# saegsali/visual-odometry-project

Measured on AMD Instinct MI355X. Metric: VO frames/sec at 1376x1241, 2k keypoints; pose err vs reference, higher is better.
Workload: dtype f64

## Files before the change

### include/vo_hip.h

```cpp
#ifndef VO_HIP_H
#define VO_HIP_H

#include <stddef.h>
#include <stdint.h>

#ifdef __cplusplus
extern "C" {
#endif

typedef struct vo_ctx vo_ctx;

typedef enum vo_status {
  VO_OK = 0,
  VO_EINVAL = -1,
  VO_ENOMEM = -2,
  VO_EHIP = -3,
  VO_ECAPACITY = -4,
  VO_ETRACKING = -5
} vo_status;


int vo_create(int device, void* stream, vo_ctx** out);
void vo_destroy(vo_ctx* ctx);
const char* vo_last_error(const vo_ctx* ctx);
// ... 229 lines not shown
int vo_ransac_replay(vo_ransac_state* st, const uint8_t* valid, const int32_t* counts, int B,
                     int N, int64_t* n_done, int32_t* best_count, int32_t* best_idx,
                     int idx_offset, int* consumed, int* finished);

typedef struct vo_pipeline vo_pipeline;
typedef struct vo_pipeline_config {
  int32_t H, W, n_frames;
  int32_t n_keypoints, harris_patch, nms_radius;
  double harris_kappa;
  int32_t klt_win, klt_max_level, klt_max_iter, hyp;
  double klt_eps, klt_min_eig, klt_err_threshold;
  double p3p_thr_sq, ransac_outlier_ratio, ransac_confidence;
  int64_t ransac_max_iterations;
  double K[9];
  double Kinv[9];
  int32_t refine_iters;
  int32_t feature_cap;
  double bearing_threshold;
  double redetect_fraction;
  int32_t debug_fault_every;
  int32_t redetect_start_pose;
  double detect_margin;
  int32_t debug_never_detect;
  double detect_losses;
  int32_t sequences;
  int32_t tracker_mode;
  int32_t sift_cap;
  int32_t track_ids;
  double match_ratio;
  int32_t detector;
  int32_t st_block;
  double st_quality;
  double st_min_distance;
} vo_pipeline_config;
typedef struct vo_step_result {
  double R[9], t[3];
  int32_t n_tracked;
  int32_t n_inliers;
  int32_t best_index;
  int32_t hyp_valid;
  int64_t ransac_iterations;
  int32_t draws_consumed;
  int32_t refine_iterations;
  double R_refined[9], t_refined[3];
  double refine_cost;
  int32_t n_features_in;
// ... 209 lines not shown
```

### visual-odometry-project_amd/csrc/harris.hip

```cpp
#include "vo_internal.h"

#pragma clang fp contract(off)

namespace {

constexpr int NT = 256;
constexpr int RX = 64;
constexpr int RY = 32;

struct resp_geom {
  int pr, GW, GWp, GH, IWp, IH;
};
typedef short pk16 __attribute__((ext_vector_type(2)));
__device__ __forceinline__ pk16 as_pk16(unsigned v) { return __builtin_bit_cast(pk16, v); }
__device__ __forceinline__ unsigned as_u32(pk16 v) { return __builtin_bit_cast(unsigned, v); }
__host__ __device__ inline resp_geom response_geometry(int p) {
  resp_geom g;
  g.pr = p >> 1;
  g.GW = RX + 2 * g.pr;
  g.GWp = (g.GW + 3) & ~3;
  g.GH = RY + 2 * g.pr;
  g.IWp = g.GWp + 4;
  g.IH = g.GH + 2;
  return g;
// ... 1334 lines not shown
      VO_HIP_TRY(ctx, hipFuncSetAttribute(reinterpret_cast<const void*>(&harris_response_kernel<0>),
                                          hipFuncAttributeMaxDynamicSharedMemorySize, (int)response_lds_bytes(31)));
      lds_opt_in = true;
    }
    vo_prof_scope ps(ctx, VO_K_HARRIS_RESPONSE);
    if (patch == 9)
      hipLaunchKernelGGL(harris_response_kernel<9>, grid, dim3(NT), lds, ctx->stream, d_img, H, W, patch, kappa,
                         d_scores, img_stride, d_go);
    else
      hipLaunchKernelGGL(harris_response_kernel<0>, grid, dim3(NT), lds, ctx->stream, d_img, H, W, patch, kappa,
                         d_scores, img_stride, d_go);
  }
  return vo_check_launch(ctx, "harris_response_kernel");
}

extern "C" {

int vo_nms_keypoints_dev(vo_ctx* ctx, const double* d_scores, int H, int W, int N, int r, double* d_kp_xy) {
  return vo_nms_keypoints_batch_dev(ctx, d_scores, 1, H, W, N, r, d_kp_xy, 0);
}

}

int vo_nms_keypoints_batch_dev(vo_ctx* ctx, const double* d_scores, int S, int H, int W, int N, int r, double* d_kp_xy,
                               size_t kp_stride, const int* d_go) {
  if (!ctx) return VO_EINVAL;
  VO_REQUIRE(ctx, S >= 1 && S <= 65535, "nms: bad sequence count");
  VO_REQUIRE(ctx, d_scores && d_kp_xy, "nms: null pointer");
  VO_REQUIRE(ctx, H > 0 && W > 0 && (int64_t)H * W < (1ll << 30), "nms: bad map size %dx%d", W, H);
  VO_REQUIRE(ctx, W < 65536 && H < 65536, "nms: map side must be < 65536");
  VO_REQUIRE(ctx, N >= 1 && N <= MAX_N, "nms: N must be in 1..%d", MAX_N);
  VO_REQUIRE(ctx, r >= 0 && r <= 12, "nms: radius must be in 0..12");
  VO_HIP_TRY(ctx, hipSetDevice(ctx->device));
  const unsigned cap = (unsigned)H * (unsigned)W;
  const unsigned cap_c = next_pow2(2u * cap);
  const dim3 grid(vo_cdiv(W, CX), vo_cdiv(H, CY), S);
  const unsigned nblk = grid.x * grid.y;
  const size_t seg_total = (size_t)nblk * SEG;
  const size_t Sz = (size_t)S;
  VO_TRY(vo_ensure(ctx, ctx->nms_keys_l1, Sz * seg_total * 8));
  VO_TRY(vo_ensure(ctx, ctx->nms_idx_l1, Sz * seg_total * 4));
  VO_TRY(vo_ensure(ctx, ctx->nms_keys_a1, Sz * seg_total * 8));
  VO_TRY(vo_ensure(ctx, ctx->nms_idx_a1, Sz * seg_total * 4));
  VO_TRY(vo_ensure(ctx, ctx->nms_cand, Sz * seg_total * 4));
  VO_TRY(vo_ensure(ctx, ctx->nms_segcnt, Sz * nblk * sizeof(uint4)));
  VO_TRY(vo_ensure(ctx, ctx->nms_keys_c, Sz * cap_c * 8));
  VO_TRY(vo_ensure(ctx, ctx->nms_idx_c, Sz * cap_c * 4));
  VO_TRY(vo_ensure(ctx, ctx->nms_sel, Sz * MAX_N * 4));
  if (ctx->nms_hist.cap < Sz * 2 * HIST_TOTAL * 4 || ctx->nms_S != S) {
    VO_TRY(vo_ensure(ctx, ctx->nms_hist, Sz * 2 * HIST_TOTAL * 4));
    VO_HIP_TRY(ctx, hipMemsetAsync(ctx->nms_hist.p, 0, ctx->nms_hist.cap, ctx->stream));
    ctx->nms_S = S;
  }
  if (ctx->nms_rank.cap < Sz * RANK_MAX * 4) {
    VO_TRY(vo_ensure(ctx, ctx->nms_rank, Sz * RANK_MAX * 4));
    VO_HIP_TRY(ctx, hipMemsetAsync(ctx->nms_rank.p, 0, ctx->nms_rank.cap, ctx->stream));
// ... 13 lines not shown
    B.alive = cap;
    B.hist = HIST_TOTAL;
    B.rank = RANK_MAX;
    B.sel = MAX_N;
    B.kp = kp_stride;
  }
  B.go = d_go;
  nms_ctl* ctl = (nms_ctl*)ctx->nms_ctl.p;

  unsigned long long* keys_l1 = (unsigned long long*)ctx->nms_keys_l1.p;
  unsigned long long* keys_a1 = (unsigned long long*)ctx->nms_keys_a1.p;
  unsigned* idx_l1 = (unsigned*)ctx->nms_idx_l1.p;
  unsigned* idx_a1 = (unsigned*)ctx->nms_idx_a1.p;
  unsigned long long* keys_c = (unsigned long long*)ctx->nms_keys_c.p;
  unsigned* idx_c = (unsigned*)ctx->nms_idx_c.p;
  unsigned* cand = (unsigned*)ctx->nms_cand.p;
  uint4* segcnt = (uint4*)ctx->nms_segcnt.p;
  unsigned* alive = (unsigned*)ctx->nms_alive.p;
  ctx->nms_parity ^= 1;
  unsigned* hist = (unsigned*)ctx->nms_hist.p + (size_t)ctx->nms_parity * Sz * HIST_TOTAL;
  unsigned* hist_other = (unsigned*)ctx->nms_hist.p + (size_t)(1 - ctx->nms_parity) * Sz * HIST_TOTAL;
  unsigned* rank = (unsigned*)ctx->nms_rank.p;
  hipStream_t st = ctx->stream;
  {
    bool& lds_opt_in = ctx->lds_opt_in[1];
    if (!lds_opt_in) {
      const int max_dyn = (int)candidates_lds_bytes(12);
      VO_HIP_TRY(ctx, hipFuncSetAttribute(reinterpret_cast<const void*>(&nms_candidates_kernel<5>),
                                          hipFuncAttributeMaxDynamicSharedMemorySize, max_dyn));
      VO_HIP_TRY(ctx, hipFuncSetAttribute(reinterpret_cast<const void*>(&nms_candidates_kernel<0>),
                                          hipFuncAttributeMaxDynamicSharedMemorySize, max_dyn));
      lds_opt_in = true;
    }
    vo_prof_scope ps(ctx, VO_K_NMS_CANDIDATES);
    const size_t lds = candidates_lds_bytes(r);
    if (r == 5)
      hipLaunchKernelGGL(nms_candidates_kernel<5>, grid, dim3(NT), lds, st, d_scores, H, W, r, keys_l1, idx_l1,
                         keys_a1, idx_a1, segcnt, hist, ctl, B);
    else
      hipLaunchKernelGGL(nms_candidates_kernel<0>, grid, dim3(NT), lds, st, d_scores, H, W, r, keys_l1, idx_l1,
                         keys_a1, idx_a1, segcnt, hist, ctl, B);
  }
  VO_TRY(vo_check_launch(ctx, "nms_candidates_kernel"));
  ctx->nms_alive_dirty = true;
  {
    vo_prof_scope ps(ctx, VO_K_NMS_COMPACT);
    hipLaunchKernelGGL(nms_compact_kernel, dim3(nblk, S), dim3(NT), 0, st, keys_l1, idx_l1, keys_a1, idx_a1, segcnt,
                       cand, keys_c, idx_c, alive, ctl, cap_c, hist, hist_other, N, B);
  }
  VO_TRY(vo_check_launch(ctx, "nms_compact_kernel"));
  const size_t round_lds = (size_t)((CX + 2 * r) | 1) * ((CY + 2 * r) + CY) * 4;
  {
    vo_prof_scope ps(ctx, VO_K_NMS_ROUND);
    const dim3 g(nblk, S), b(RT);
    if (r == 5)
      hipLaunchKernelGGL((nms_round_kernel<5, true>), g, b, round_lds, st, d_scores, alive, segcnt, cand, keys_c,
                         idx_c, ctl, cap_c, H, W, r, (int)grid.x, B);
    else
      hipLaunchKernelGGL((nms_round_kernel<0, true>), g, b, round_lds, st, d_scores, alive, segcnt, cand, keys_c,
                         idx_c, ctl, cap_c, H, W, r, (int)grid.x, B);
  }
  VO_TRY(vo_check_launch(ctx, "nms_round_kernel"));
  {
    vo_prof_scope ps(ctx, VO_K_NMS_RANK);
    hipLaunchKernelGGL(nms_rank_kernel, dim3(RK_BLOCKS, S), dim3(NT), 0, st, keys_c, idx_c, ctl, rank, alive, segcnt,
                       cand, nblk, B);
  }
// ... 146 lines not shown
```

### visual-odometry-project_amd/csrc/pipeline.h

```cpp
#pragma once

#include <linux/futex.h>
#include <sys/prctl.h>
#include <sys/syscall.h>
#include <time.h>
#include <unistd.h>

#include <atomic>
#include <chrono>
#include <cmath>
#include <cstdlib>
#include <string>
#include <mutex>
#include <thread>
#include <vector>

#include "vo_state.h"
#include "state_device.h"

struct vo_pipeline_boot;

struct vo_pipeline {
  vo_ctx* ctx = nullptr;
  vo_ctx* det = nullptr;
  vo_ctx* trk = nullptr;
  hipEvent_t evKlt[2] = {nullptr, nullptr}, evRegroup[2] = {nullptr, nullptr};
  vo_pipeline_config cfg;
  std::vector<vo_cam> cams;
  vo_cam* d_cams = nullptr;
  std::vector<char> idle;
  vo_pcg64 seed_rng;
  int n_levels = 1, cap = 0, words = 0, S = 1;
  size_t px = 0, pyr_bytes = 0;
  uint8_t* d_img = nullptr;
  uint8_t* d_pyr = nullptr;
  double* d_kp = nullptr;
  double* d_scores[2] = {nullptr, nullptr};
  int* d_det_go = nullptr;
  float* d_st_xy = nullptr;
  int32_t* d_st_n = nullptr;
  int32_t* d_det_cnt = nullptr;
  int st_rounds = 0;
  double detect_limit = 0.0;
  double detect_losses = 2.5;
  hipEvent_t evPyr[3] = {nullptr, nullptr, nullptr}, evDet[3] = {nullptr, nullptr, nullptr};
  std::vector<uint8_t*> h_img;
  std::vector<hipEvent_t> evImg;
  hipStream_t up_stream = nullptr;
  std::vector<hipEvent_t> evUp;
  std::vector<char> pinned, plain_used;
  std::vector<int> n_pinned;
  struct lens_t {
    bool on = false, have_raw = false;
    double dist[5] = {0, 0, 0, 0, 0}, K_raw[9] = {0, 0, 0, 0, 0, 0, 0, 0, 0};
  };
  std::vector<lens_t> lens;
  uint8_t* d_raw[2] = {nullptr, nullptr};
  uint8_t* h_bgr = nullptr;
  hipEvent_t evBgr = nullptr;
  int prepared_idx = -1, prepared_slot = -1;
  int slot = 0, det_flip = 0, prev_frame = -1;
  vo_feat F[2];
  void* feat_mem = nullptr;
  int cur = 0;
  vo_seq_ctl* d_ctl = nullptr;
  float *d_next = nullptr, *d_err = nullptr;
  uint8_t* d_status = nullptr;
// ... 144 lines not shown
  }
}

static inline vo_cam make_cam(const double* K, const double* Kinv) {
  vo_cam c;
  memcpy(c.K, K, sizeof(c.K));
  if (Kinv) {
    memcpy(c.Kinv, Kinv, sizeof(c.Kinv));
  } else {
    const double fx = K[0], fy = K[4], cx = K[2], cy = K[5];
    const double ki[9] = {1.0 / fx, 0.0, -cx / fx, 0.0, 1.0 / fy, -cy / fy, 0.0, 0.0, 1.0};
    memcpy(c.Kinv, ki, sizeof(ki));
  }
  return c;
}

#define VO_PIPE_INTERNAL __attribute__((visibility("hidden")))
VO_PIPE_INTERNAL void worker_main(vo_pipeline* p);
VO_PIPE_INTERNAL int worker_idle(vo_pipeline* p);
VO_PIPE_INTERNAL int prime(vo_pipeline* p, bool wait = true, int q0 = 0, int Sn = 0);
VO_PIPE_INTERNAL void vo_pipeline_boot_free(vo_pipeline* p);
VO_PIPE_INTERNAL void vo_structure_loop_free(vo_pipeline* p);
VO_PIPE_INTERNAL int vo_structure_loop_requeue(vo_pipeline* p, int q, long k);
VO_PIPE_INTERNAL int enqueue_detection(vo_pipeline* p, int frame, int s, bool force, char* err_buf = nullptr, int q0 = 0, int Sn = 0);
```

### visual-odometry-project_amd/csrc/pipeline.hip

```cpp
#include "pipeline.h"

#pragma clang fp contract(off)

namespace {

hipError_t mset(hipStream_t st, void* dst, int v, size_t bytes) {
  hipError_t e = hipMemsetAsync(dst, v, bytes, st);
  return e != hipSuccess ? e : hipStreamSynchronize(st);
}

uint32_t next_pow2(uint64_t v) {
  uint32_t r = 1;
  while (r < v) r <<= 1;
  return r;
}

vo_feat carve(char*& q, int cap, int S, bool ids) {
  vo_feat f;
  auto take = [&](size_t bytes) {
    void* r = q;
    q += (bytes * S + 255) & ~size_t(255);
    return r;
  };
  f.kp = (float*)take((size_t)cap * 8);
// ... 170 lines not shown
  }
  const int cap = cfg->feature_cap > 0 ? cfg->feature_cap : 2 * cfg->n_keypoints;
  VO_REQUIRE(ctx, cap >= cfg->n_keypoints && cap <= 32768, "pipeline: feature_cap must be in n_keypoints..32768");
  VO_HIP_TRY(ctx, hipSetDevice(ctx->device));
  vo_pipeline* p = new (std::nothrow) vo_pipeline();
  if (!p) return VO_ENOMEM;
  p->ctx = ctx;
  p->cfg = *cfg;
  p->cap = cap;
  p->words = vo_cdiv(cap, 64);
  p->S = cfg->sequences > 0 ? cfg->sequences : 1;
  p->cfg.sequences = p->S;
  const int S = p->S;
  if (p->cfg.bearing_threshold == 0.0) p->cfg.bearing_threshold = 0.0075;
  if (p->cfg.redetect_fraction == 0.0) p->cfg.redetect_fraction = 0.8;
  if (p->cfg.detect_margin == 0.0) p->cfg.detect_margin = 0.01;
  if (p->cfg.detect_losses <= 0.0) p->cfg.detect_losses = 2.5;
  if (p->cfg.st_block == 0) p->cfg.st_block = 7;
  if (p->cfg.st_quality == 0.0) p->cfg.st_quality = 0.01;
  if (p->cfg.st_min_distance == 0.0) p->cfg.st_min_distance = 8.0;
  p->detect_losses = p->cfg.detect_losses;
  p->detect_limit = p->cfg.detect_margin < 0.0 ? -1.0 : p->cfg.redetect_fraction + p->cfg.detect_margin;
  if (p->cfg.debug_never_detect) p->detect_limit = 0.0;
  {
    bool given = false;
    for (double v : cfg->Kinv) given |= v != 0.0;
    p->cams.assign((size_t)p->S, make_cam(cfg->K, given ? cfg->Kinv : nullptr));
  }
  p->idle.assign((size_t)p->S, 0);
  memset(&p->seed_rng, 0, sizeof(p->seed_rng));
  int rc = VO_OK;
  void* side = getenv("VO_ONE_STREAM") ? (void*)ctx->stream : nullptr;
  {
    const char* sc = getenv("VO_SIDE_CUS");
    p->side_cfg = vo_stream_cfg_parse(sc, getenv("VO_STREAM_PRIORITY"));
    if (!sc && p->S <= 2 && p->detect_limit >= 0.0 && !side && cfg->tracker_mode == 0) {
      hipDeviceProp_t prop;
      if (hipGetDeviceProperties(&prop, ctx->device) == hipSuccess && prop.multiProcessorCount >= 128) {
        p->side_cfg.cu_lo = 32;
        p->side_cfg.cu_hi = prop.multiProcessorCount - 1;
      }
    }
    if (!side && side_pool_evicts()) side_evict_except(ctx->device, p->side_cfg);
    for (vo_ctx** c : {&p->trk, &p->det})
      if ((side ? vo_create_stream(ctx->device, side, p->side_cfg, c) : side_take(ctx->device, p->side_cfg, c)) != VO_OK)
        rc = vo_set_error(ctx, VO_EHIP, "pipeline: cannot create the side streams");
// ... 357 lines not shown
```

### visual-odometry-project_amd/csrc/pipeline_step.hip

```cpp
#include "pipeline.h"

#pragma clang fp contract(off)

namespace {

__global__ __launch_bounds__(64) void detect_decide_kernel(const vo_seq_ctl* __restrict__ ctl, int S, double limit, int n_det,
                                                           int force, int* __restrict__ go, double losses) {
  const int q = blockIdx.x * 64 + threadIdx.x;
  if (q >= S) return;
  if (ctl[q].fault & VO_FAULT_IDLE) {
    go[q] = 0;
    return;
  }
  const int n2 = ctl[q].n2;
  const int lost = max(ctl[q].n_in - (ctl[q].redetected ? (n_det < 0 ? ctl[q].num_features : n_det) : 0) - n2, 0);
  go[q] = (force || limit < 0.0 || (limit > 0.0 && (double)n2 - losses * (double)lost < (double)ctl[q].num_features * limit)) ? 1 : 0;
}

__global__ void ctl_resume_kernel(vo_seq_ctl* __restrict__ ctl) {
  ctl->fault = 0;
  ctl->n_p3p = ctl->n_tri;
}

__global__ __launch_bounds__(256) void sift_kp_f64_kernel(const float* __restrict__ rows, const int* __restrict__ n, int cap,
// ... 45 lines not shown
}

void copy_prof(vo_ctx* q, const vo_ctx* from) {
  q->prof_on = from->prof_on;
  q->prof_kernel = from->prof_kernel;
  q->prof_every = from->prof_every;
}

void sync_prof(vo_pipeline* p) {
  for (vo_ctx* q : {p->det, p->trk}) copy_prof(q, p->ctx);
}

}

static int launch_error(vo_pipeline* p, char* err_buf, int rc, const char* what, const char* detail) {
  if (err_buf) {
    snprintf(err_buf, 256, "%s: %s", what, detail);
    return rc;
  }
  return vo_set_error(p->ctx, rc, "%s: %s", what, detail);
}


int enqueue_detection(vo_pipeline* p, int frame, int s, bool force, char* err_buf, int q0, int Sn) {
  const vo_pipeline_config& c = p->cfg;
  if (Sn <= 0) Sn = p->S - q0;
  p->det_flip ^= 1;
  vo_ctx* det = p->det;
  double* scores = p->d_scores[p->det_flip];
  det->nms_kp_f32 = nullptr;
  int* go = p->d_det_go + (size_t)s * p->S + q0;
  bool wait_ok = hipStreamWaitEvent(det->stream, p->evImg[frame], 0) == hipSuccess;
  if (wait_ok && p->n_pinned[frame] > 0) wait_ok = hipStreamWaitEvent(det->stream, p->evUp[frame], 0) == hipSuccess;
  if (!wait_ok) return launch_error(p, err_buf, VO_EHIP, "detection", "hipStreamWaitEvent failed");
  hipLaunchKernelGGL(detect_decide_kernel, dim3(vo_cdiv(Sn, 64)), dim3(64), 0, det->stream, p->d_ctl + q0, Sn, p->detect_limit,
                     c.detector == 1 ? -1 : c.n_keypoints, force ? 1 : 0, go, p->detect_losses);
  int rc = vo_check_launch(det, "detect_decide_kernel");
  if (c.detector == 1) {
    vo_prof_scope ps(det, VO_K_SHI_TOMASI_CHAIN);
    const int N = c.n_keypoints;
    float* xy = p->d_st_xy + (size_t)q0 * N * 2;
    int32_t *n = p->d_st_n + q0, *over = p->d_st_n + p->S + q0;
    if (rc == VO_OK)
      rc = vo_good_features_batch_gated_dev(det, p->img(q0, frame), p->img_stride(), Sn, c.H, c.W, nullptr, 0, N, c.st_quality,
                                            c.st_min_distance, c.st_block, xy, (size_t)N, n, over, nullptr, p->st_rounds,
                                            VO_GFB_CANDIDATES, go);
    if (rc == VO_OK) {
      hipLaunchKernelGGL(st_close_kernel, dim3(vo_cdiv(N, 256), Sn), dim3(256), 0, det->stream, (const float*)xy, (size_t)N * 2,
                         (const int32_t*)n, (const int32_t*)over, (const int*)go, N, p->kp(q0, s), p->det_stride(),
                         p->d_det_cnt + (size_t)s * p->S + q0);
      rc = vo_check_launch(det, "st_close_kernel");
    }
    if (rc == VO_OK && hipEventRecord(p->evDet[s], det->stream) != hipSuccess) rc = VO_EHIP;
    return rc != VO_OK ? launch_error(p, err_buf, rc, "detection", vo_last_error(det)) : VO_OK;
  }
  if (rc == VO_OK)
    rc = vo_harris_response_batch_dev(det, p->img(q0, frame), p->img_stride(), Sn, c.H, c.W, c.harris_patch, c.harris_kappa,
                                      scores, go);
  if (rc == VO_OK)
    rc = vo_nms_keypoints_batch_dev(det, scores, Sn, c.H, c.W, c.n_keypoints, c.nms_radius, p->kp(q0, s), p->det_stride(),
                                    go);
  if (rc == VO_OK && hipEventRecord(p->evDet[s], det->stream) != hipSuccess) rc = VO_EHIP;
  return rc != VO_OK ? launch_error(p, err_buf, rc, "detection", vo_last_error(det)) : VO_OK;
}

static int enqueue_pyramid(vo_pipeline* p, int frame, int s, int q0 = 0, int Sn = 0) {
  if (s == p->prepared_slot) p->prepared_idx = p->prepared_slot = -1;
  if (p->n_pinned[frame] > 0 && hipStreamWaitEvent(p->trk->stream, p->evUp[frame], 0) != hipSuccess)
    return vo_set_error(p->ctx, VO_EHIP, "pyramid: hipStreamWaitEvent failed");
  const vo_pipeline_config& c = p->cfg;
  if (Sn <= 0) Sn = p->S - q0;
  for (int a = q0; a < q0 + Sn;) {
    if (p->idle[a]) {
      ++a;
      continue;
    }
    int b = a + 1;
    while (b < q0 + Sn && !p->idle[b]) ++b;
    const int rc = vo_pyramid_build_batch_dev(p->trk, p->img(a, frame), p->img_stride(), b - a, c.H, c.W, p->n_levels,
                                              p->pyr(a, s), p->pyr_stride());
    if (rc != VO_OK) return vo_set_error(p->ctx, rc, "pyramid: %s", vo_last_error(p->trk));
    a = b;
  }
  VO_HIP_TRY(p->ctx, hipEventRecord(p->evPyr[s], p->trk->stream));
// ... 100 lines not shown
  }
  return VO_OK;
}

static int enqueue_pose_half(vo_pipeline* p, const vo_pipeline::flight_t& f, int q0, int Sn, unsigned seq);

static int enqueue_chain(vo_pipeline* p, const vo_pipeline::flight_t& f, bool first_half_only, int debug_fault_every,
                         int q0, int Sn, unsigned seq) {
  vo_ctx* ctx = p->ctx;
  const vo_pipeline_config& c = p->cfg;
  const size_t q = (size_t)q0;
  const vo_feat A = vo_feat_seq(p->F[f.fcur], q), B = vo_feat_seq(p->F[1 - f.fcur], q);
  vo_seq_ctl* ctl = p->d_ctl + q0;
  VO_HIP_TRY(ctx, hipStreamWaitEvent(ctx->stream, p->evKlt[f.k & 1], 0));
  vo_append ap;
  ap.det_kp = p->kp(q0, f.a);
  ap.det_stride = p->det_stride();
  ap.n_det = c.n_keypoints;
  ap.frac = c.redetect_fraction;
  ap.pose_mode = c.redetect_start_pose;
  ap.debug_fault_every = debug_fault_every > 0 ? debug_fault_every : 0;
  ap.det_go = p->d_det_go + (size_t)f.a * p->S + q0;
  ap.nf_par = (int)(f.k & 1);
  if (p->d_det_cnt) ap.n_det_dev = p->d_det_cnt + (size_t)f.a * p->S + q0;
  ctx->next_stop = p->evRegroup[f.k & 1];
  VO_TRY(vo_state_regroup_klt(ctx, ctl, A, B, p->d_next + q * p->cap * 2, p->d_status + q * p->cap, p->d_err + q * p->cap,
                              (float)c.klt_err_threshold, ap, p->cap, Sn));
  if (first_half_only) return VO_OK;
  return enqueue_pose_half(p, f, q0, Sn, seq);
}

static int enqueue_pose_half(vo_pipeline* p, const vo_pipeline::flight_t& f, int q0, int Sn, unsigned seq) {
  vo_ctx* ctx = p->ctx;
  const int debug_pose_fault = p->pose_fault_hook && p->cfg.debug_fault_every < 0 ? -p->cfg.debug_fault_every : 0;
  const vo_pipeline_config& c = p->cfg;
  const size_t q = (size_t)q0;
  const vo_feat B = vo_feat_seq(p->F[1 - f.fcur], q);
  vo_seq_ctl* ctl = p->d_ctl + q0;
  vo_hyp_batch hb;
  hb.S = Sn;
  hb.X = (size_t)p->cap * 3;
  hb.x = (size_t)p->cap * 2;
  hb.raws = p->ring_len;
  hb.ctl = sizeof(vo_seq_ctl);
  hb.cam = reinterpret_cast<const double*>(p->d_cams + q);
  hb.cam_stride = sizeof(vo_cam) / sizeof(double);
// ... 106 lines not shown
  (void)hipSetDevice(p->ctx->device);
  unsigned seen = 0;
  long idle = 0;
  double idle_since = 0.0;
  for (;;) {
    if (p->job_posted.load(std::memory_order_acquire) == seen) {
      if (p->quit.load(std::memory_order_acquire)) return;
      if (idle == 0) idle_since = now_s();
      if ((++idle & 63) != 0 || now_s() - idle_since < p->spin_s) {
        __builtin_ia32_pause();
      } else {
        p->worker_asleep.store(1, std::memory_order_seq_cst);
        if (p->job_posted.load(std::memory_order_seq_cst) == seen && !p->quit.load(std::memory_order_seq_cst))
          futex_wait(&p->job_posted, seen);
        p->worker_asleep.store(0, std::memory_order_seq_cst);
        idle = 0;
      }
      continue;
    }
    idle = 0;
    const vo_pipeline::flight_t j = p->jobs[seen & 3];
    const int rc = p->cfg.tracker_mode == 1   ? enqueue_sift(p, j, p->worker_err)
                   : p->cfg.tracker_mode == 2 ? enqueue_harris_front(p, j, p->worker_err)
                                              : enqueue_detection(p, j.next_idx, j.b, false, p->worker_err);
    if (rc != VO_OK) p->worker_rc = rc;
    ++seen;
    p->job_done.store(seen, std::memory_order_release);
  }
}

static int worker_check(vo_pipeline* p) {
  if (p->worker_rc != VO_OK) {
    const int rc = p->worker_rc;
    p->worker_rc = VO_OK;
    return vo_set_error(p->ctx, rc, "%s", p->worker_err);
  }
  return VO_OK;
}

int worker_idle(vo_pipeline* p) {
  if (p->threads_budget < 2) return VO_OK;
  const unsigned posted = p->job_posted.load(std::memory_order_relaxed);
  wait_until(50e-6, [&] { return p->job_done.load(std::memory_order_acquire) == posted; });
  return worker_check(p);
}

int prime(vo_pipeline* p, bool wait, int q0, int Sn) {
// ... 105 lines not shown
      const unsigned my = p->job_posted.load(std::memory_order_relaxed);
      wait_until(50e-6, [&] { return (int)(p->job_done.load(std::memory_order_acquire) - my) >= 0; });
      VO_TRY(worker_check(p));
      sync_prof(p);
      if (detect_early) post_job(p, f);
    } else {
      sync_prof(p);
    }
    double tn = now_s();
    p->dbg_part[0] += tn - tq;
    tq = tn;
    const bool have_pyr = p->prepared_idx == next_idx && p->prepared_slot == f.b;
    p->prepared_idx = p->prepared_slot = -1;
    VO_TRY(enqueue_tracker(p, f, !have_pyr, 0, p->S));
    tn = now_s();
    p->dbg_part[1] += tn - tq;
    tq = tn;
    for (int q = 0; q < p->S; ++q) VO_TRY(ensure_raws(p, q));
    tn = now_s();
    p->dbg_part[2] += tn - tq;
    tq = tn;
    VO_TRY(enqueue_chain(p, f, false, c.debug_fault_every, 0, p->S, f.seq));
    for (int q = 0; q < p->S; ++q) p->slot_seq[(size_t)f.rslot * p->S + q] = f.seq;
    if (p->threads_budget < 2) VO_TRY(enqueue_detection(p, f.next_idx, f.b, false));
    else if (!detect_early) post_job(p, f);
    p->dbg_part[3] += now_s() - tq;
    p->flight[p->n_flight++] = f;
  }
  ++p->steps_submitted;
  p->slot = f.b;
  p->cur = 1 - f.fcur;
  p->prev_frame = next_idx;
  p->dbg_submit += now_s() - t_in;
  ++p->dbg_steps;
  return VO_OK;
}

}

static void record_words(const vo_step_result* rec, unsigned seq, unsigned* head, unsigned* tail) {
  const unsigned* dw = reinterpret_cast<const unsigned*>(rec);
  unsigned x = 0u, y = 0u;
  for (size_t k = 0; k + 2 < sizeof(*rec) / 4; ++k) {
    x ^= dw[k];
    y += vo_state_dev::record_mix(dw[k], (int)k);
  }
  *head = seq ^ x;
// ... 288 lines not shown
```

### visual-odometry-project_amd/csrc/state.hip

```cpp
#include <cmath>

#include "dlt_device.h"
#include "state_device.h"

#pragma clang fp contract(off)

namespace {

constexpr int RG_T = 1024;


using namespace vo_state_dev;

__device__ __forceinline__ unsigned long long block_scan_excl(unsigned long long v, unsigned long long* s_wave,
                                                              unsigned long long* total) {
  const int lane = threadIdx.x & 63, wv = threadIdx.x >> 6, nw = blockDim.x >> 6;
  unsigned long long inc = v;
#pragma unroll
  for (int off = 1; off < 64; off <<= 1) {
    const unsigned long long o = __shfl_up(inc, off);
    if (lane >= off) inc += o;
  }
  if (lane == 63) s_wave[wv] = inc;
  __syncthreads();
// ... 253 lines not shown
    r_e[u] = err[min(j, capm)];
    r_st[u] = A.state[min(j, pitm)];
  }
  const int jo = start + tid, jq = min(jo, pitm), jx = min(jo, capm);
  double o_land[3], o_track[2], o_kp[2], o_pose[12];
  const float o_nx = next_xy[2 * jx];
  const float o_ny = next_xy[2 * jx + 1];
#pragma unroll
  for (int k = 0; k < 3; ++k) o_land[k] = A.land[3 * jq + k];
#pragma unroll
  for (int k = 0; k < 2; ++k) {
    o_track[k] = A.track[2 * jq + k];
    o_kp[k] = A.kp64[2 * jq + k];
  }
#pragma unroll
  for (int k = 0; k < 12; ++k) o_pose[k] = A.pose[(size_t)k * A.pitch + jq];
  int2 o_id = make_int2(0, 0);
  if (IDS) o_id = A.ids[jq];
  auto key_of = [&](int j) -> int {
    const int jc = min(j, n_in - 1), js = min(j, max(n - 1, 0));
    const int s8 = status[jc];
    const float e = err[jc];
    const int st_raw = A.state[js];
    const int keep = (int)(j < n_in) & (int)(s8 != 0) & (int)(e < err_thr);
    const int st = j < n ? st_raw : 0;
    return keep ? (st == 2 ? 0 : (st == 1 ? 1 : 2)) : 3;
  };
  unsigned long long c_all = 0ull, c_before = 0ull;
  int my_key = 3;
  for (int base0 = 0; base0 < n_in; base0 += 256 * RG_U) {
    int keys[RG_U];
#pragma unroll
    for (int u = 0; u < RG_U; ++u) {
      const int j = base0 + u * 256 + tid;
      if (base0 == 0) {
        const int keep = (int)(j < n_in) & (int)(r_s8[u] != 0) & (int)(r_e[u] < err_thr);
        const int st = j < n ? r_st[u] : 0;
        keys[u] = keep ? (st == 2 ? 0 : (st == 1 ? 1 : 2)) : 3;
      } else {
        keys[u] = key_of(j);
      }
    }
#pragma unroll
    for (int u = 0; u < RG_U; ++u) {
      const int base = base0 + u * 256;
      const int key = keys[u];
      if (base == start) my_key = key;
      if (key < 3) {
        const unsigned long long one = 1ull << (21 * key);
        c_all += one;
        if (base < start) c_before += one;
      }
    }
  }
#pragma unroll
  for (int off = 32; off >= 1; off >>= 1) {
    c_all += __shfl_xor(c_all, off);
    c_before += __shfl_xor(c_before, off);
  }
// ... 52 lines not shown
      B.state[dst] = 1;
      B.land[3 * dst] = B.land[3 * dst + 1] = B.land[3 * dst + 2] = dnan();
      B.track[2 * dst] = (double)(float)ap.det_kp[2 * d];
      B.track[2 * dst + 1] = (double)(float)ap.det_kp[2 * d + 1];
#pragma unroll
      for (int k = 0; k < 12; ++k)
        B.pose[(size_t)k * B.pitch + dst] = ap.pose_mode ? ctl->T_wc[k] : ((k == 0 || k == 5 || k == 10) ? 1.0 : 0.0);
    }
  }
  if (blockIdx.x == 0 && tid == 0) {
    ctl->n_in = n_in;
    ctl->redetected = redetect ? 1 : 0;
    ctl->det_ran = ap.det_go ? ap.det_go[blockIdx.y] : 1;
    if (ap.n_det_dev) {
      const int nf_next = redetect ? n_det : nf;
      ctl->nf[ap.nf_par ^ 1] = nf_next;
      ctl->num_features = nf_next;
    }
    if (IDS) {
      ctl->next_id[ap.nf_par ^ 1] = nid + (n_in - n);
      ctl->id_step[ap.nf_par ^ 1] = step_k + 1;
    }
    ctl->n2 = T0 + T1 + T2;
    ctl->n_tri = T0;
    ctl->n_mat = T1;
    ctl->n_new = T2;
    const int few = T0 < 8 ? VO_FAULT_FEW_LANDMARKS : 0;
    ctl->n_p3p = few ? 0 : T0;
    ctl->few = few;
  }
}


__global__ __launch_bounds__(256) void state_candidates_kernel(vo_seq_ctl* __restrict__ ctl, vo_feat B,
                                                               const unsigned long long* __restrict__ best_mask,
                                                               const vo_cam* __restrict__ cams, double bearing_thr, int use_refined,
                                                               int words) {
  if (blockIdx.y != 0) {
    const size_t q = blockIdx.y;
    ctl += q;
    B = vo_feat_seq(B, q);
    best_mask += q * (size_t)words;
  }
  const vo_cam& cam = cams[blockIdx.y];
  if (ctl->fault) return;
  const int tid = threadIdx.x;
// ... 409 lines not shown
```

### visual-odometry-project_amd/csrc/state_device.h

```cpp
#pragma once
#include <cstddef>
#include "vo_state.h"

#pragma clang fp contract(off)

namespace vo_state_dev {

__device__ __forceinline__ double dnan() { return __longlong_as_double(0x7ff8000000000000ll); }

__device__ __forceinline__ void rigid_inverse_3x4(const double* T, double* Ti) {
#pragma unroll
  for (int r = 0; r < 3; ++r) {
#pragma unroll
    for (int c = 0; c < 3; ++c) Ti[4 * r + c] = T[4 * c + r];
    Ti[4 * r + 3] = -(T[r] * T[3] + T[4 + r] * T[7] + T[8 + r] * T[11]);
  }
}

__device__ __forceinline__ void k_times(const double* K, const double* T, double* C) {
#pragma unroll
  for (int r = 0; r < 3; ++r)
#pragma unroll
    for (int c = 0; c < 4; ++c) C[4 * r + c] = K[3 * r] * T[c] + K[3 * r + 1] * T[4 + c] + K[3 * r + 2] * T[8 + c];
}

__host__ __device__ inline long long table_lookup(const double* table, int len, long long max_it, double orat) {
  int lo = 0, hi = len;
  while (lo < hi) {
    const int mid = (lo + hi) >> 1;
    if (table[1 + mid] <= orat) lo = mid + 1;
    else hi = mid;
// ... 331 lines not shown
```

### visual-odometry-project_amd/csrc/vo_internal.h

```cpp
#pragma once
#include <hip/hip_runtime.h>
#include <hip/hip_ext.h>

#include <cstdarg>
#include <cstdint>
#include <cstdio>
#include <cstdlib>
#include <cstring>
#include <vector>

#include "vo_hip.h"

struct vo_buf {
  void* p = nullptr;
  size_t cap = 0;
};

struct vo_prof_slot {
  double total_ms = 0.0;
  int64_t launches = 0;
};

struct vo_prof_pair {
  int k;
// ... 4 lines not shown
  int device = 0;
  hipStream_t stream = nullptr;
  bool own_stream = false;
  char err[512] = {0};
  hipEvent_t next_stop = nullptr;

  bool prof_on = false;
  int prof_kernel = -1;
  int prof_every = 1;
  unsigned prof_seen[VO_K_COUNT] = {0};
  vo_prof_slot prof[VO_K_COUNT];
  std::vector<hipEvent_t> ev_free;
  typedef vo_prof_pair pending_ev;
  std::vector<pending_ev> ev_pending;

  vo_buf img, img2, scores, kp, desc;
  vo_buf nms_keys_l1, nms_idx_l1, nms_keys_a1, nms_idx_a1;
  vo_buf nms_keys_c, nms_idx_c;
  vo_buf nms_hist, nms_ctl, nms_sel, nms_cand, nms_alive, nms_segcnt, nms_rank;
  bool nms_alive_dirty = false;
  int nms_parity = 0;
  int nms_S = 0;
  float* nms_kp_f32 = nullptr;
  vo_buf scratch[16];
  vo_buf match_arrived;
  int match_last_path = -1;
  bool lds_opt_in[2] = {false, false};
  hipStream_t aux_stream = nullptr;
  hipStream_t aux_stream2 = nullptr;
  std::vector<hipEvent_t> aux_events;
  vo_buf sift_arena;
  void* h_pin = nullptr;
  size_t h_pin_cap = 0;
  int64_t bytes_h2d = 0, bytes_d2h = 0;
  vo_buf f8_ctl, f8_raws, f8_F, f8_counts, f8_risky, f8_masks, f8_table, f8_samples;
  std::vector<double> f8_table_host;
  double f8_table_conf = 0.0;
  vo_buf ba_work, ba_match;
};

template <class K, class... A>
inline void vo_launch_stop(vo_ctx* ctx, K kernel, dim3 grid, dim3 block, size_t lds, hipStream_t st, A... args) {
  if (ctx->next_stop) {
    hipExtLaunchKernelGGL(kernel, grid, block, (unsigned)lds, st, nullptr, ctx->next_stop, 0, args...);
    ctx->next_stop = nullptr;
  } else {
// ... 164 lines not shown
  int32_t* best = nullptr;
};
int vo_essential_hypotheses_dev(vo_ctx* ctx, const double* d_x1, const double* d_x2, int N, const double* K1, const double* K2,
                                const int32_t* samples, int Hyp, int error_kind, double threshold, const vo_e5_work& w,
                                int32_t* best_count, int32_t* best_sol, uint8_t* valid);
int vo_essential_ransac_dev(vo_ctx* ctx, const double* d_x1, const double* d_x2, int N, const double* K1, const double* K2,
                            int error_kind, double threshold, double outlier_ratio, double confidence, int64_t max_iterations,
                            vo_pcg64* rng, double* d_E, uint8_t* d_inl, int64_t* iterations, int32_t* best_count);
int vo_triangulate_dlt_ndev(vo_ctx* ctx, const double* d_x1, const double* d_x2, const int32_t* d_n, int n_cap,
                            const double* d_C1, const double* d_C2, double* d_X);
int vo_refine_pose_ndev(vo_ctx* ctx, const double* d_X, const double* d_x, int N, const int32_t* d_n, const double* K,
                        const uint8_t* d_mask8, const uint64_t* d_mask_bits, const double* d_Rt0, int max_iter,
                        double* d_out14, unsigned tag);
struct vo_klt_source {
  const int32_t* n = nullptr;
  const int32_t* num_features = nullptr;
  double frac = 0.0;
  const double* det_kp = nullptr;
  int n_det = 0;
  unsigned long long* ts = nullptr;
  const int* det_go = nullptr;
  const int32_t* n_det_dev = nullptr;
};
struct vo_klt_batch {
  int S = 1;
  size_t pyr = 0;
  size_t xy = 0;
  size_t out = 0;
  size_t ctl = 0;
  size_t det = 0;
};
int vo_klt_track_ndev(vo_ctx* ctx, const uint8_t* d_prev, const uint8_t* d_prev_pyr, const uint8_t* d_next,
                      const uint8_t* d_next_pyr, int H, int W, int n_levels, const float* d_prev_xy, int N,
                      const int32_t* d_n, int win, int max_iter, double eps, double min_eig, float* d_next_xy,
                      uint8_t* d_status, float* d_err, const vo_klt_source* src = nullptr,
                      const vo_klt_batch* batch = nullptr, double fb_max = 0.0, float* d_fb = nullptr);
int vo_pyramid_build_batch_dev(vo_ctx* ctx, const uint8_t* d_img, size_t img_stride, int S, int H, int W, int n_levels,
                               uint8_t* d_pyr, size_t pyr_stride);
int vo_harris_response_batch_dev(vo_ctx* ctx, const uint8_t* d_img, size_t img_stride, int S, int H, int W, int patch,
                                 double kappa, double* d_scores, const int* d_go = nullptr);
int vo_nms_keypoints_batch_dev(vo_ctx* ctx, const double* d_scores, int S, int H, int W, int N, int r, double* d_kp_xy,
                               size_t kp_stride, const int* d_go = nullptr);
```

### visual-odometry-project_amd/csrc/vo_state.h

```cpp
#pragma once
#include "vo_internal.h"

struct vo_feat {
  float* kp;
  double* kp64;
  uint8_t* state;
  uint8_t* cand;
  double* land;
  double* track;
  double* pose;
  int pitch;
  int2* ids = nullptr;
};

__host__ __device__ inline vo_feat vo_feat_seq(vo_feat F, size_t q) {
  const size_t n = q * (size_t)F.pitch;
  F.kp += 2 * n;
  F.kp64 += 2 * n;
  F.state += n;
  F.cand += n;
  F.land += 3 * n;
  F.track += 2 * n;
  F.pose += 12 * n;
  if (F.ids) F.ids += n;
// ... 20 lines not shown
  int32_t n2, n_tri, n_mat, n_new;
  int32_t n_p3p;
  int32_t fault;
  int32_t step;
  int32_t solve_flag;
  int32_t few;
  int32_t cont;
  int64_t n_iterations;
  double outlier_ratio;
  uint64_t raw_pos;
  int64_t n_iterations0;
  double outlier_ratio0;
  int32_t best_idx, best_count, consumed, hyp_valid;
  int64_t n_done;
  int32_t n_cand, n_dropped, n_land, done;
  int32_t n_pend, pad_pend;
  double best_pose[12];
  double refined[16];
  double T_cw[12], T_wc[12], T_cw_prev[12], T_wc_prev[12], T_in_cw[12], T_in_wc[12];
  unsigned long long ts[8];
  int32_t nf[2];
  int32_t next_id[2];
  int32_t id_step[2];
};

struct vo_cam {
  double K[9], Kinv[9];
};

struct vo_append {
  const double* det_kp;
  size_t det_stride;
  int n_det;
  double frac;
  int pose_mode;
  int debug_fault_every;
  const int* det_go;
  const int32_t* n_det_dev = nullptr;
  int nf_par = 0;
};

struct vo_replay_args {
  const uint8_t* valid;
  const int32_t* counts;
  const double *R, *t;
  const unsigned long long* masks;
  int words, hyp;
  const double* table;
  int table_len;
  long long max_it;
  unsigned long long* best_mask;
};

struct vo_pose_job {
  vo_seq_ctl* ctl;
  vo_replay_args rp;
  int do_replay;
  vo_feat B;
  const vo_cam* cam;
  double bearing_thr;
  int max_iter;
  int tail;
// ... 33 lines not shown
```

### visual-odometry-project_amd/vo/_native.py

```python
import ctypes as C
import atexit
import os
import threading
import weakref

import numpy as np

_LIB_PATH = os.path.join(os.path.dirname(os.path.abspath(__file__)), "lib", "libvo_hip.so")

VO_OK, VO_EINVAL, VO_ENOMEM, VO_EHIP, VO_ECAPACITY, VO_ETRACKING = 0, -1, -2, -3, -4, -5
_CODES = {VO_EINVAL: "VO_EINVAL", VO_ENOMEM: "VO_ENOMEM", VO_EHIP: "VO_EHIP", VO_ECAPACITY: "VO_ECAPACITY",
          VO_ETRACKING: "VO_ETRACKING"}

K_HARRIS_RESPONSE, K_NMS_CANDIDATES, K_NMS_THRESHOLD, K_NMS_COMPACT, K_NMS_SELECT = 0, 1, 2, 3, 4
K_PATCH_DESC, K_PYR_DOWN, K_KLT_TRACK, K_DLT, K_P3P_SOLVE, K_P3P_SCORE, K_REPROJ, K_MATCH = 5, 6, 7, 8, 9, 10, 11, 12
K_SHI_TOMASI_CHAIN = 27
K_WINDOW_BA, K_WINDOW_BUILD = 28, 29
K_TWOVIEW_HYP, K_TWOVIEW_SCORE = 30, 31
K_WINDOW_STRUCTURE = 32
K_LOOP_RECORD, K_LOOP_JOIN, K_LOOP_WRITE = 33, 34, 35
K_BRIEF_DESCRIBE, K_HAMMING_KNN2 = 36, 37
K_COUNT = 38


# ... 24 lines not shown
        st["state"]["state"] = (self.state_hi << 64) | self.state_lo
        st["state"]["inc"] = (self.inc_hi << 64) | self.inc_lo
        st["has_uint32"] = int(self.has_uint32)
        st["uinteger"] = int(self.uinteger)
        gen.bit_generator.state = st


class RansacState(C.Structure):
    _fields_ = [("outlier_ratio", C.c_double), ("confidence", C.c_double), ("max_iterations", C.c_int64),
                ("n_iterations", C.c_int64), ("s", C.c_int32), ("adaptive", C.c_int32)]


class PipelineConfig(C.Structure):
    _fields_ = [("H", C.c_int32), ("W", C.c_int32), ("n_frames", C.c_int32),
                ("n_keypoints", C.c_int32), ("harris_patch", C.c_int32), ("nms_radius", C.c_int32),
                ("harris_kappa", C.c_double),
                ("klt_win", C.c_int32), ("klt_max_level", C.c_int32), ("klt_max_iter", C.c_int32), ("hyp", C.c_int32),
                ("klt_eps", C.c_double), ("klt_min_eig", C.c_double), ("klt_err_threshold", C.c_double),
                ("p3p_thr_sq", C.c_double), ("ransac_outlier_ratio", C.c_double), ("ransac_confidence", C.c_double),
                ("ransac_max_iterations", C.c_int64),
                ("K", C.c_double * 9), ("Kinv", C.c_double * 9), ("refine_iters", C.c_int32), ("feature_cap", C.c_int32),
                ("bearing_threshold", C.c_double), ("redetect_fraction", C.c_double),
                ("debug_fault_every", C.c_int32), ("redetect_start_pose", C.c_int32), ("detect_margin", C.c_double),
                ("debug_never_detect", C.c_int32), ("detect_losses", C.c_double), ("sequences", C.c_int32),
                ("tracker_mode", C.c_int32), ("sift_cap", C.c_int32), ("track_ids", C.c_int32),
                ("match_ratio", C.c_double),
                ("detector", C.c_int32), ("st_block", C.c_int32), ("st_quality", C.c_double),
                ("st_min_distance", C.c_double)]


class StepResult(C.Structure):
    _fields_ = [("R", C.c_double * 9), ("t", C.c_double * 3), ("n_tracked", C.c_int32), ("n_inliers", C.c_int32),
                ("best_index", C.c_int32), ("hyp_valid", C.c_int32), ("ransac_iterations", C.c_int64),
                ("draws_consumed", C.c_int32), ("refine_iterations", C.c_int32),
                ("R_refined", C.c_double * 9), ("t_refined", C.c_double * 3), ("refine_cost", C.c_double),
                ("n_features_in", C.c_int32), ("redetected", C.c_int32), ("n_triangulated", C.c_int32),
                ("n_candidates", C.c_int32), ("n_dropped", C.c_int32), ("n_landmarks", C.c_int32),
                ("fault", C.c_int32), ("recovered", C.c_int32), ("detector_ran", C.c_int32), ("reserved", C.c_int32),
                ("raw_pos", C.c_uint64), ("T_wc", C.c_double * 12),
                ("ts", C.c_uint64 * 8), ("seq_head", C.c_uint32), ("seq_tail", C.c_uint32)]

    def pose_world_cam(self):
        return np.vstack([np.array(self.T_wc).reshape(3, 4), [0.0, 0.0, 0.0, 1.0]])

    @property
    def idle(self):
        return self.n_features_in == -1
# ... 1165 lines not shown
```

### visual-odometry-project_amd/vo/_pipeline.py

```python
import ctypes as C

import numpy as np


def _ptr(a):
    return a.ctypes.data_as(C.c_void_p) if a is not None else None


def _c(a, dtype):
    return np.ascontiguousarray(a, dtype=dtype)


def _as_4x4(pose):
    pose = np.asarray(pose, np.float64)
    if pose.shape == (3, 4):
        pose = np.vstack([pose, [0.0, 0.0, 0.0, 1.0]])
    return np.ascontiguousarray(pose)


DETECTORS = {"harris": 0, "shi-tomasi": 1}

TRACK_ROW = np.dtype([("id", "<i4"), ("born", "<i4"), ("x", "<f4"), ("y", "<f4"), ("state", "<i4"), ("candidate", "<i4"),
                      ("X", "<f8"), ("Y", "<f8"), ("Z", "<f8")])
TRACK_HEADER = np.dtype([("n", "<i4"), ("step", "<i4"), ("next_id", "<i4"), ("seq", "<i4")])
# ... 3 lines not shown
    n = step = next_id = seq = 0

    def __array_finalize__(self, obj):
        for k in ("n", "step", "next_id", "seq"):
            setattr(self, k, getattr(obj, k, 0))

    @classmethod
    def from_bytes(cls, raw, cap):
        raw = np.ascontiguousarray(raw, np.uint8)
        head = raw[:16].view(TRACK_HEADER)[0]
        m = max(0, min(int(head["n"]), int(cap)))
        rec = raw[16:16 + 48 * m].view(TRACK_ROW).copy().view(cls)
        rec.n, rec.step, rec.next_id, rec.seq = (int(head[k]) for k in ("n", "step", "next_id", "seq"))
        return rec


class Pipeline:
    def __init__(self, ctx, H, W, n_frames, K, n_keypoints=2000, harris_patch=9, harris_kappa=0.09, nms_radius=5,
                 klt_win=15, klt_max_level=2, klt_max_iter=10, klt_eps=0.03, klt_min_eig=1e-4,
                 klt_err_threshold=100.0, hyp=1000, p3p_threshold=1.0, outlier_ratio=0.9, confidence=0.99,
                 max_iterations=1000, seed=2023, refine_iters=0, feature_cap=0, bearing_threshold=0.0075,
                 redetect_fraction=0.8, debug_fault_every=0, redetect_start_pose="identity", sequences=1,
                 detect_margin=0.01, debug_never_detect=0, detect_losses=2.5, tracker="klt", sift_cap=0, match_ratio=0.0,
                 detector="harris", st_quality=0.0, st_min_distance=0.0, st_block=0, track_ids=False):
        from vo import _native
        self.ctx = ctx
        self.cfg = _native.PipelineConfig()
        c = self.cfg
        c.H, c.W, c.n_frames = H, W, n_frames
        c.n_keypoints, c.harris_patch, c.nms_radius, c.harris_kappa = n_keypoints, harris_patch, nms_radius, harris_kappa
        c.klt_win, c.klt_max_level, c.klt_max_iter, c.hyp = klt_win, klt_max_level, klt_max_iter, hyp
        c.klt_eps, c.klt_min_eig, c.klt_err_threshold = klt_eps, klt_min_eig, klt_err_threshold
        c.p3p_thr_sq = p3p_threshold
        c.ransac_outlier_ratio, c.ransac_confidence = outlier_ratio, confidence
        c.ransac_max_iterations = -1 if max_iterations is None or max_iterations == np.inf else int(max_iterations)
        c.refine_iters = int(refine_iters)
        c.feature_cap = int(feature_cap)
        c.bearing_threshold = float(bearing_threshold)
        c.redetect_fraction = float(redetect_fraction)
        c.debug_fault_every = int(debug_fault_every)
        c.redetect_start_pose = {"identity": 0, "current": 1}[redetect_start_pose]
        c.sequences = int(sequences)
        c.detect_margin = float(detect_margin)
        c.debug_never_detect = int(debug_never_detect)
        c.detect_losses = float(detect_losses)
        c.tracker_mode = {"klt": 0, "sift": 1, "harris": 2}[tracker]
        c.sift_cap = int(sift_cap)
        c.match_ratio = float(match_ratio)
        c.detector = DETECTORS[detector]
        c.st_quality, c.st_min_distance, c.st_block = float(st_quality), float(st_min_distance), int(st_block)
        c.track_ids = 1 if track_ids else 0
        self.track_ids = bool(track_ids)
        self.detector = detector
        self.tracker = tracker
        self.sequences = int(sequences)
        K = np.asarray(K, np.float64).reshape(3, 3)
        self.K = K
        for i, v in enumerate(K.reshape(9)):
            c.K[i] = v
        for i, v in enumerate(np.linalg.inv(K).reshape(9)):
            c.Kinv[i] = v
        h = C.c_void_p()
        ctx._chk(ctx._lib.vo_pipeline_create(ctx._h, C.byref(c), C.byref(h)))
        self._h = h
        self._pinned_src = {}
        ctx._pipelines.add(self)
        self.cap = ctx._lib.vo_pipeline_feature_cap(self._h)
        self.seed(np.random.default_rng(seed))

    def close(self):
        if getattr(self, "_h", None):
            if getattr(self, "_loop", None):
                self._loop.close()
            self.ctx._lib.vo_pipeline_destroy(self._h)
# ... 291 lines not shown
```

Baseline: 10920.

## Cancel speculative keypoint detection on device once tracking count confirms no redetect

Adds a device-side recheck kernel that runs during the NMS stage of speculative detection. It reads a tagged tracked-feature count, written atomically by the regroup kernel, and clears the per-sequence go flag when the tracked count is no longer below the redetect fraction. Downstream NMS compact and round kernels can then skip work for detections that are not needed. The cost is extra tiny kernel launches, a new control field, and cross-stream relaxed atomics whose timing determines whether any skipping happens.

```diff
diff --git a/include/vo_hip.h b/include/vo_hip.h
--- a/include/vo_hip.h
+++ b/include/vo_hip.h
@@ -275,6 +275,7 @@
   int32_t redetect_start_pose;
   double detect_margin;
   int32_t debug_never_detect;
+  int32_t detect_confirm;
   double detect_losses;
   int32_t sequences;
   int32_t tracker_mode;
diff --git a/visual-odometry-project_amd/csrc/harris.hip b/visual-odometry-project_amd/csrc/harris.hip
--- a/visual-odometry-project_amd/csrc/harris.hip
+++ b/visual-odometry-project_amd/csrc/harris.hip
@@ -1380,6 +1380,28 @@
 
 }
 
+namespace {
+
+__global__ __launch_bounds__(64) void det_recheck_kernel(vo_det_recheck rc, int S) {
+  const int q = blockIdx.x * 64 + threadIdx.x;
+  if (q >= S || !rc.go[q]) return;
+  const unsigned long long word = __hip_atomic_load(
+      reinterpret_cast<const unsigned long long*>(reinterpret_cast<const char*>(rc.tag) + (size_t)q * rc.stride), __ATOMIC_RELAXED,
+      __HIP_MEMORY_SCOPE_AGENT);
+  if ((unsigned)(word >> 32) != rc.want) return;
+  const int m = (int)(unsigned)(word & 0xffffffffull);
+  const int nf = *reinterpret_cast<const int32_t*>(reinterpret_cast<const char*>(rc.num_features) + (size_t)q * rc.stride);
+  if (!((double)m < (double)nf * rc.frac)) rc.go[q] = 0;
+}
+
+int launch_recheck(vo_ctx* ctx, const vo_det_recheck* rc, int S) {
+  if (!rc || !rc->go) return VO_OK;
+  hipLaunchKernelGGL(det_recheck_kernel, dim3(vo_cdiv(S, 64)), dim3(64), 0, ctx->stream, *rc, S);
+  return vo_check_launch(ctx, "det_recheck_kernel");
+}
+
+}
+
 int vo_nms_keypoints_batch_dev(vo_ctx* ctx, const double* d_scores, int S, int H, int W, int N, int r, double* d_kp_xy,
                                size_t kp_stride, const int* d_go) {
   if (!ctx) return VO_EINVAL;
@@ -1390,6 +1412,8 @@
   VO_REQUIRE(ctx, N >= 1 && N <= MAX_N, "nms: N must be in 1..%d", MAX_N);
   VO_REQUIRE(ctx, r >= 0 && r <= 12, "nms: radius must be in 0..12");
   VO_HIP_TRY(ctx, hipSetDevice(ctx->device));
+  const vo_det_recheck* recheck = ctx->nms_recheck;
+  ctx->nms_recheck = nullptr;
   const unsigned cap = (unsigned)H * (unsigned)W;
   const unsigned cap_c = next_pow2(2u * cap);
   const dim3 grid(vo_cdiv(W, CX), vo_cdiv(H, CY), S);
@@ -1449,6 +1473,7 @@
   unsigned* hist_other = (unsigned*)ctx->nms_hist.p + (size_t)(1 - ctx->nms_parity) * Sz * HIST_TOTAL;
   unsigned* rank = (unsigned*)ctx->nms_rank.p;
   hipStream_t st = ctx->stream;
+  VO_TRY(launch_recheck(ctx, recheck, S));
   {
     bool& lds_opt_in = ctx->lds_opt_in[1];
     if (!lds_opt_in) {
@@ -1470,6 +1495,7 @@
   }
   VO_TRY(vo_check_launch(ctx, "nms_candidates_kernel"));
   ctx->nms_alive_dirty = true;
+  VO_TRY(launch_recheck(ctx, recheck, S));
   {
     vo_prof_scope ps(ctx, VO_K_NMS_COMPACT);
     hipLaunchKernelGGL(nms_compact_kernel, dim3(nblk, S), dim3(NT), 0, st, keys_l1, idx_l1, keys_a1, idx_a1, segcnt,
diff --git a/visual-odometry-project_amd/csrc/pipeline.h b/visual-odometry-project_amd/csrc/pipeline.h
--- a/visual-odometry-project_amd/csrc/pipeline.h
+++ b/visual-odometry-project_amd/csrc/pipeline.h
@@ -43,6 +43,7 @@
   int st_rounds = 0;
   double detect_limit = 0.0;
   double detect_losses = 2.5;
+  bool confirm_on = false;
   hipEvent_t evPyr[3] = {nullptr, nullptr, nullptr}, evDet[3] = {nullptr, nullptr, nullptr};
   std::vector<uint8_t*> h_img;
   std::vector<hipEvent_t> evImg;
@@ -233,4 +234,5 @@
 VO_PIPE_INTERNAL void vo_pipeline_boot_free(vo_pipeline* p);
 VO_PIPE_INTERNAL void vo_structure_loop_free(vo_pipeline* p);
 VO_PIPE_INTERNAL int vo_structure_loop_requeue(vo_pipeline* p, int q, long k);
-VO_PIPE_INTERNAL int enqueue_detection(vo_pipeline* p, int frame, int s, bool force, char* err_buf = nullptr, int q0 = 0, int Sn = 0);
+VO_PIPE_INTERNAL int enqueue_detection(vo_pipeline* p, int frame, int s, bool force, char* err_buf = nullptr, int q0 = 0, int Sn = 0,
+                                       unsigned recheck = 0u);
diff --git a/visual-odometry-project_amd/csrc/pipeline.hip b/visual-odometry-project_amd/csrc/pipeline.hip
--- a/visual-odometry-project_amd/csrc/pipeline.hip
+++ b/visual-odometry-project_amd/csrc/pipeline.hip
@@ -216,6 +216,7 @@
   p->detect_losses = p->cfg.detect_losses;
   p->detect_limit = p->cfg.detect_margin < 0.0 ? -1.0 : p->cfg.redetect_fraction + p->cfg.detect_margin;
   if (p->cfg.debug_never_detect) p->detect_limit = 0.0;
+  p->confirm_on = p->cfg.detect_confirm >= 0 && p->cfg.tracker_mode == 0 && p->cfg.detector == 0 && p->detect_limit > 0.0;
   {
     bool given = false;
     for (double v : cfg->Kinv) given |= v != 0.0;
diff --git a/visual-odometry-project_amd/csrc/pipeline_step.hip b/visual-odometry-project_amd/csrc/pipeline_step.hip
--- a/visual-odometry-project_amd/csrc/pipeline_step.hip
+++ b/visual-odometry-project_amd/csrc/pipeline_step.hip
@@ -91,7 +91,7 @@
 }
 
 
-int enqueue_detection(vo_pipeline* p, int frame, int s, bool force, char* err_buf, int q0, int Sn) {
+int enqueue_detection(vo_pipeline* p, int frame, int s, bool force, char* err_buf, int q0, int Sn, unsigned recheck) {
   const vo_pipeline_config& c = p->cfg;
   if (Sn <= 0) Sn = p->S - q0;
   p->det_flip ^= 1;
@@ -126,9 +126,20 @@
   if (rc == VO_OK)
     rc = vo_harris_response_batch_dev(det, p->img(q0, frame), p->img_stride(), Sn, c.H, c.W, c.harris_patch, c.harris_kappa,
                                       scores, go);
+  vo_det_recheck look;
+  if (recheck != 0u && p->confirm_on && !force) {
+    look.go = go;
+    look.tag = &p->d_ctl[q0].trk_tag;
+    look.num_features = &p->d_ctl[q0].num_features;
+    look.stride = sizeof(vo_seq_ctl);
+    look.want = recheck;
+    look.frac = c.redetect_fraction;
+    det->nms_recheck = &look;
+  }
   if (rc == VO_OK)
     rc = vo_nms_keypoints_batch_dev(det, scores, Sn, c.H, c.W, c.n_keypoints, c.nms_radius, p->kp(q0, s), p->det_stride(),
                                     go);
+  det->nms_recheck = nullptr;
   if (rc == VO_OK && hipEventRecord(p->evDet[s], det->stream) != hipSuccess) rc = VO_EHIP;
   return rc != VO_OK ? launch_error(p, err_buf, rc, "detection", vo_last_error(det)) : VO_OK;
 }
@@ -275,6 +286,7 @@
   ap.debug_fault_every = debug_fault_every > 0 ? debug_fault_every : 0;
   ap.det_go = p->d_det_go + (size_t)f.a * p->S + q0;
   ap.nf_par = (int)(f.k & 1);
+  ap.tag = p->confirm_on ? f.seq : 0u;
   if (p->d_det_cnt) ap.n_det_dev = p->d_det_cnt + (size_t)f.a * p->S + q0;
   ctx->next_stop = p->evRegroup[f.k & 1];
   VO_TRY(vo_state_regroup_klt(ctx, ctl, A, B, p->d_next + q * p->cap * 2, p->d_status + q * p->cap, p->d_err + q * p->cap,
@@ -427,7 +439,7 @@
     const vo_pipeline::flight_t j = p->jobs[seen & 3];
     const int rc = p->cfg.tracker_mode == 1   ? enqueue_sift(p, j, p->worker_err)
                    : p->cfg.tracker_mode == 2 ? enqueue_harris_front(p, j, p->worker_err)
-                                              : enqueue_detection(p, j.next_idx, j.b, false, p->worker_err);
+                                              : enqueue_detection(p, j.next_idx, j.b, false, p->worker_err, 0, 0, j.seq);
     if (rc != VO_OK) p->worker_rc = rc;
     ++seen;
     p->job_done.store(seen, std::memory_order_release);
@@ -579,7 +591,7 @@
     tq = tn;
     VO_TRY(enqueue_chain(p, f, false, c.debug_fault_every, 0, p->S, f.seq));
     for (int q = 0; q < p->S; ++q) p->slot_seq[(size_t)f.rslot * p->S + q] = f.seq;
-    if (p->threads_budget < 2) VO_TRY(enqueue_detection(p, f.next_idx, f.b, false));
+    if (p->threads_budget < 2) VO_TRY(enqueue_detection(p, f.next_idx, f.b, false, nullptr, 0, 0, f.seq));
     else if (!detect_early) post_job(p, f);
     p->dbg_part[3] += now_s() - tq;
     p->flight[p->n_flight++] = f;
diff --git a/visual-odometry-project_amd/csrc/state.hip b/visual-odometry-project_amd/csrc/state.hip
--- a/visual-odometry-project_amd/csrc/state.hip
+++ b/visual-odometry-project_amd/csrc/state.hip
@@ -299,7 +299,7 @@
     const int s8 = status[jc];
     const float e = err[jc];
     const int st_raw = A.state[js];
-    const int keep = (int)(j < n_in) & (int)(s8 != 0) & (int)(e < err_thr);
+    const int keep = (int)(j < n_in) & klt_kept(s8, e, err_thr);
     const int st = j < n ? st_raw : 0;
     return keep ? (st == 2 ? 0 : (st == 1 ? 1 : 2)) : 3;
   };
@@ -311,7 +311,7 @@
     for (int u = 0; u < RG_U; ++u) {
       const int j = base0 + u * 256 + tid;
       if (base0 == 0) {
-        const int keep = (int)(j < n_in) & (int)(r_s8[u] != 0) & (int)(r_e[u] < err_thr);
+        const int keep = (int)(j < n_in) & klt_kept(r_s8[u], r_e[u], err_thr);
         const int st = j < n ? r_st[u] : 0;
         keys[u] = keep ? (st == 2 ? 0 : (st == 1 ? 1 : 2)) : 3;
       } else {
@@ -410,6 +410,9 @@
       ctl->id_step[ap.nf_par ^ 1] = step_k + 1;
     }
     ctl->n2 = T0 + T1 + T2;
+    if (ap.tag)
+      __hip_atomic_store(&ctl->trk_tag, ((unsigned long long)ap.tag << 32) | (unsigned)(T0 + T1 + T2), __ATOMIC_RELAXED,
+                         __HIP_MEMORY_SCOPE_AGENT);
     ctl->n_tri = T0;
     ctl->n_mat = T1;
     ctl->n_new = T2;
diff --git a/visual-odometry-project_amd/csrc/state_device.h b/visual-odometry-project_amd/csrc/state_device.h
--- a/visual-odometry-project_amd/csrc/state_device.h
+++ b/visual-odometry-project_amd/csrc/state_device.h
@@ -7,6 +7,8 @@
 namespace vo_state_dev {
 
 __device__ __forceinline__ double dnan() { return __longlong_as_double(0x7ff8000000000000ll); }
+
+__device__ __forceinline__ int klt_kept(int status, float err, float err_thr) { return (int)(status != 0) & (int)(err < err_thr); }
 
 __device__ __forceinline__ void rigid_inverse_3x4(const double* T, double* Ti) {
 #pragma unroll
diff --git a/visual-odometry-project_amd/csrc/vo_internal.h b/visual-odometry-project_amd/csrc/vo_internal.h
--- a/visual-odometry-project_amd/csrc/vo_internal.h
+++ b/visual-odometry-project_amd/csrc/vo_internal.h
@@ -50,6 +50,7 @@
   int nms_parity = 0;
   int nms_S = 0;
   float* nms_kp_f32 = nullptr;
+  struct vo_det_recheck* nms_recheck = nullptr;
   vo_buf scratch[16];
   vo_buf match_arrived;
   int match_last_path = -1;
@@ -260,6 +261,14 @@
   const int* det_go = nullptr;
   const int32_t* n_det_dev = nullptr;
 };
+struct vo_det_recheck {
+  int* go = nullptr;
+  const unsigned long long* tag = nullptr;
+  const int32_t* num_features = nullptr;
+  size_t stride = 0;
+  unsigned want = 0;
+  double frac = 0.0;
+};
 struct vo_klt_batch {
   int S = 1;
   size_t pyr = 0;
diff --git a/visual-odometry-project_amd/csrc/vo_state.h b/visual-odometry-project_amd/csrc/vo_state.h
--- a/visual-odometry-project_amd/csrc/vo_state.h
+++ b/visual-odometry-project_amd/csrc/vo_state.h
@@ -66,6 +66,7 @@
   int32_t nf[2];
   int32_t next_id[2];
   int32_t id_step[2];
+  unsigned long long trk_tag;
 };
 
 struct vo_cam {
@@ -82,6 +83,7 @@
   const int* det_go;
   const int32_t* n_det_dev = nullptr;
   int nf_par = 0;
+  unsigned tag = 0;
 };
 
 struct vo_replay_args {
diff --git a/visual-odometry-project_amd/vo/_native.py b/visual-odometry-project_amd/vo/_native.py
--- a/visual-odometry-project_amd/vo/_native.py
+++ b/visual-odometry-project_amd/vo/_native.py
@@ -70,7 +70,7 @@
                 ("K", C.c_double * 9), ("Kinv", C.c_double * 9), ("refine_iters", C.c_int32), ("feature_cap", C.c_int32),
                 ("bearing_threshold", C.c_double), ("redetect_fraction", C.c_double),
                 ("debug_fault_every", C.c_int32), ("redetect_start_pose", C.c_int32), ("detect_margin", C.c_double),
-                ("debug_never_detect", C.c_int32), ("detect_losses", C.c_double), ("sequences", C.c_int32),
+                ("debug_never_detect", C.c_int32), ("detect_confirm", C.c_int32), ("detect_losses", C.c_double), ("sequences", C.c_int32),
                 ("tracker_mode", C.c_int32), ("sift_cap", C.c_int32), ("track_ids", C.c_int32),
                 ("match_ratio", C.c_double),
                 ("detector", C.c_int32), ("st_block", C.c_int32), ("st_quality", C.c_double),
diff --git a/visual-odometry-project_amd/vo/_pipeline.py b/visual-odometry-project_amd/vo/_pipeline.py
--- a/visual-odometry-project_amd/vo/_pipeline.py
+++ b/visual-odometry-project_amd/vo/_pipeline.py
@@ -49,7 +49,8 @@
                  max_iterations=1000, seed=2023, refine_iters=0, feature_cap=0, bearing_threshold=0.0075,
                  redetect_fraction=0.8, debug_fault_every=0, redetect_start_pose="identity", sequences=1,
                  detect_margin=0.01, debug_never_detect=0, detect_losses=2.5, tracker="klt", sift_cap=0, match_ratio=0.0,
-                 detector="harris", st_quality=0.0, st_min_distance=0.0, st_block=0, track_ids=False):
+                 detector="harris", st_quality=0.0, st_min_distance=0.0, st_block=0, track_ids=False,
+                 detect_confirm=True):
         from vo import _native
         self.ctx = ctx
         self.cfg = _native.PipelineConfig()
@@ -77,6 +78,7 @@
         c.detector = DETECTORS[detector]
         c.st_quality, c.st_min_distance, c.st_block = float(st_quality), float(st_min_distance), int(st_block)
         c.track_ids = 1 if track_ids else 0
+        c.detect_confirm = 0 if detect_confirm else -1
         self.track_ids = bool(track_ids)
         self.detector = detector
         self.tracker = tracker
```

New measurement: 10830. Within noise of the previous version (-0.8%).
